# ashvardanian/StringWars

Measured on AMD Instinct MI355X. Metric: GCUPS (DP cell updates/s) batched Levenshtein, higher is better.
Workload: dtype u32; 1 GPU; C2 tokens64: 1000000 ASCII token pairs per GPU, lengths U[32,96], unbounded Levenshtein, tapes prepared and resident in HBM; step=one synchronous call (results visible on return), pairs_per_gpu=1000000, pairs_total=1000000, cells_per_gpu=4273938131, algorithm=auto, offsets=uint32, collective=none, seed=42

## Files before the change

### stringwars_amd/csrc/bp_item.hpp

```cpp
#pragma once
#include <type_traits>

#include "common.hpp"
#include "bp_window.hpp"

namespace swh {

struct SymWindow32 {
    const uint32_t *base;
    int lo, hi;
    __device__ __forceinline__ void init(const uint32_t *data, uint64_t start, uint64_t total) {
        auto c31 = [](int64_t v) { return (int)(v < -0x40000000ll ? -0x40000000ll : (v > 0x40000000ll ? 0x40000000ll : v)); };
        base = data + start;
        lo = c31(-(int64_t)start);
        hi = c31((int64_t)total - (int64_t)start - 1);
    }
    __device__ __forceinline__ uint32_t fetch(int idx) const { return base[bp_med3i(idx, lo, hi)]; }
    __device__ __forceinline__ void fetch4(int idx, uint32_t (&out)[4]) const {
        if (hi - lo >= 3) {
            const int c = bp_med3i(idx, lo, hi - 3);
            uint4 v;
            __builtin_memcpy(&v, base + c, 16);
            out[0] = v.x; out[1] = v.y; out[2] = v.z; out[3] = v.w;
            if (__builtin_expect(c == idx, 1)) return;
        }
#pragma unroll
        for (int q = 0; q < 4; ++q) out[q] = fetch(idx + q);
    }
};

template <typename Sym> struct BpTraits;
template <> struct BpTraits<uint8_t> {
    static constexpr int kWaves = 4, kEntries = 32, kMinWavesPerSimd = 4;
};
template <> struct BpTraits<uint32_t> {
    static constexpr int kWaves = 2, kEntries = 56, kMinWavesPerSimd = 2;
};
template <typename Sym> constexpr int bp_table_words() { return BpTraits<Sym>::kEntries * 64; }
template <typename Sym> constexpr size_t bp_lds_bytes() {
    return (size_t)BpTraits<Sym>::kWaves * (bp_table_words<Sym>() + 64) * 4 + 80 * 4;
}

struct GroupTables3 {
    uint32_t tbase, mask;
    __device__ __forceinline__ void init(uint32_t *table, int lane) {
        tbase = (uint32_t)(uintptr_t)(lds_u32 *)(table + lane);
        if (tbase & 0x700u) __builtin_trap();
        mask = 0x700u;
        asm volatile("" : "+v"(mask));
    }
    template <int G> __device__ __forceinline__ uint32_t addr(uint32_t c) const {
        uint32_t s;
        if constexpr (3 * G <= 8) s = c << (8 - 3 * G);
        else s = c >> (3 * G - 8);
        return (uint32_t)__builtin_amdgcn_bitop3_b32((int)s, (int)mask, (int)tbase, 0xEA);
    }
    __device__ __forceinline__ uint32_t lookup(uint32_t c) const { return lookup_n<7>(c); }
    __device__ __forceinline__ void insert(uint32_t c, uint32_t bit) const { insert_n<7>(c, bit); }
    template <int NG, int G> __device__ __forceinline__ uint32_t entry_n(uint32_t c) const {
        if constexpr (G + 1 == NG && NG < 7) {
            uint32_t idx = c >> (3 * G);
            idx = idx < 8u ? idx : 8u;
            return *(const lds_u32 *)(uintptr_t)(tbase + (idx << 8) + 2048u * G);
        } else {
            return *(const lds_u32 *)(uintptr_t)(addr<G>(c) + 2048u * G);
        }
    }
    template <int NG> __device__ __forceinline__ uint32_t lookup_n(uint32_t c) const {
        uint32_t e = entry_n<NG, 0>(c) & entry_n<NG, 1>(c);
        e &= entry_n<NG, 2>(c) & entry_n<NG, 3>(c);
        if constexpr (NG > 4) e &= entry_n<NG, 4>(c);
        if constexpr (NG > 5) e &= entry_n<NG, 5>(c);
        if constexpr (NG > 6) e &= entry_n<NG, 6>(c);
        return e;
    }
    template <int NG> __device__ __forceinline__ void insert_n(uint32_t c, uint32_t bit) const {
        __hip_atomic_fetch_or((lds_u32 *)(uintptr_t)addr<0>(c), bit, __ATOMIC_RELAXED, __HIP_MEMORY_SCOPE_WORKGROUP);
        __hip_atomic_fetch_or((lds_u32 *)(uintptr_t)(addr<1>(c) + 2048), bit, __ATOMIC_RELAXED, __HIP_MEMORY_SCOPE_WORKGROUP);
        __hip_atomic_fetch_or((lds_u32 *)(uintptr_t)(addr<2>(c) + 4096), bit, __ATOMIC_RELAXED, __HIP_MEMORY_SCOPE_WORKGROUP);
        __hip_atomic_fetch_or((lds_u32 *)(uintptr_t)(addr<3>(c) + 6144), bit, __ATOMIC_RELAXED, __HIP_MEMORY_SCOPE_WORKGROUP);
        if constexpr (NG > 4) __hip_atomic_fetch_or((lds_u32 *)(uintptr_t)(addr<4>(c) + 8192), bit, __ATOMIC_RELAXED, __HIP_MEMORY_SCOPE_WORKGROUP);
        if constexpr (NG > 5) __hip_atomic_fetch_or((lds_u32 *)(uintptr_t)(addr<5>(c) + 10240), bit, __ATOMIC_RELAXED, __HIP_MEMORY_SCOPE_WORKGROUP);
        if constexpr (NG > 6) __hip_atomic_fetch_or((lds_u32 *)(uintptr_t)(addr<6>(c) + 12288), bit, __ATOMIC_RELAXED, __HIP_MEMORY_SCOPE_WORKGROUP);
    }
};

template <typename Sym>
struct BpWave {
    static constexpr bool kBytes = sizeof(Sym) == 1;
    uint32_t *table;
    uint32_t *acc;
    NibbleTables nib;
    GroupTables3 grp;
    int lane;
    uint64_t a_total, b_total;
    __device__ __forceinline__ void init(uint32_t *table_, uint32_t *acc_, int lane_, uint64_t a_total_, uint64_t b_total_) {
        table = table_; acc = acc_; lane = lane_; a_total = a_total_; b_total = b_total_;
        if constexpr (kBytes) nib.init(table, lane);
        else grp.init(table, lane);
#pragma unroll
        for (int k = 0; k < BpTraits<Sym>::kEntries; ++k) table[k * 64 + lane] = 0;
    }
};

template <typename Sym, bool kWide>
__device__ __forceinline__ void bp_item(const KernelArgs &args, BpWave<Sym> &wv, const uint32_t G, const bool have, const uint64_t p,
                                        const uint64_t a0, const uint32_t la, const uint64_t b0, const uint32_t lb,
                                        uint16_t *staged = nullptr, const uint64_t staged_base = 0) {
    constexpr bool kBytes = sizeof(Sym) == 1;
    constexpr bool wide_tapes = kWide;
    const int lane = wv.lane;
    uint32_t *const table = wv.table;
    uint32_t *const acc = wv.acc;
    [[maybe_unused]] const NibbleTables &nib = wv.nib;
    [[maybe_unused]] const GroupTables3 &grp = wv.grp;
    const uint64_t a_total = wv.a_total, b_total = wv.b_total;
    const uint32_t slot = (uint32_t)lane / G, blk = (uint32_t)lane - slot * G;
    const bool a_is_pattern = bp_pattern_is_a(la, lb);
    const uint32_t m = a_is_pattern ? la : lb, n = a_is_pattern ? lb : la;
    using Window = typename std::conditional<kBytes, ByteWindow, SymWindow32>::type;
    Window pat, txt;
    pat.init((const Sym *)(a_is_pattern ? args.job.a.data : args.job.b.data), a_is_pattern ? a0 : b0,
             a_is_pattern ? a_total : b_total);
    txt.init((const Sym *)(a_is_pattern ? args.job.b.data : args.job.a.data), a_is_pattern ? b0 : a0,
             a_is_pattern ? b_total : a_total);

    const uint32_t row0 = blk * 32;
    const uint32_t brows = have ? (m > row0 ? (m - row0 < 32 ? m - row0 : 32) : 0) : 0;

    constexpr int kTextRegs = kBytes ? 4 : 16;
    uint32_t tnxt[kTextRegs];
    int tshift[kBytes ? 4 : 1];
    auto fetch_text = [&](int first) {
        if constexpr (kBytes) {
            if (wide_tapes) {
                tshift[0] = txt.fetch16_raw(first, tnxt);
            } else {
#pragma unroll
                for (int q = 0; q < 4; ++q) tnxt[q] = txt.fetch4_raw(first + q * 4, tshift[q]);
            }
        } else {
#pragma unroll
            for (int q = 0; q < 16; q += 4) {
                uint32_t four[4];
                txt.fetch4(first + q, four);
#pragma unroll
                for (int r = 0; r < 4; ++r) tnxt[q + r] = four[r];
            }
        }
    };
    fetch_text(0 - (int)blk);
    [[maybe_unused]] uint32_t groups = 7;

    if constexpr (kBytes) {
        uint32_t praw[8];
        int pshift[8];
        if (wide_tapes) {
            uint32_t half[2][4];
            const int moved0 = pat.fetch16_raw((int)row0, half[0]), moved1 = pat.fetch16_raw((int)row0 + 16, half[1]);
            pat.fix16((int)row0, moved0, half[0]);
            pat.fix16((int)row0 + 16, moved1, half[1]);
#pragma unroll
            for (int q = 0; q < 8; ++q) { praw[q] = half[q >> 2][q & 3]; pshift[q] = 24; }
        } else {
#pragma unroll
            for (int q = 0; q < 8; ++q) praw[q] = pat.fetch4_raw((int)row0 + q * 4, pshift[q]);
        }
        const uint32_t row_mask = brows >= 32 ? 0xFFFFFFFFu : ((1u << brows) - 1u);
#pragma unroll
        for (int q = 0; q < 8; ++q) {
            if (brows > (uint32_t)q * 4) {
                const uint32_t dw = ByteWindow::realign(praw[q], pshift[q]);
                nib.template insert<0>(dw, row_mask & (1u << (q * 4 + 0)));
                nib.template insert<1>(dw, row_mask & (1u << (q * 4 + 1)));
                nib.template insert<2>(dw, row_mask & (1u << (q * 4 + 2)));
                nib.template insert<3>(dw, row_mask & (1u << (q * 4 + 3)));
            }
        }
    } else {
        uint32_t psym[32];
#pragma unroll
        for (int q = 0; q < 32; q += 4) {
            uint32_t four[4];
            pat.fetch4((int)row0 + q, four);
#pragma unroll
            for (int r = 0; r < 4; ++r) psym[q + r] = four[r];
        }
        uint32_t seen = 0;
#pragma unroll
        for (int q = 0; q < 32; ++q) seen |= (uint32_t)q < brows ? psym[q] : 0u;
#pragma unroll
        for (int off = 32; off >= 1; off >>= 1) seen |= (uint32_t)__shfl_xor((int)seen, off);
        groups = seen < (1u << 12) ? 4u : (seen < (1u << 15) ? 5u : (seen < (1u << 18) ? 6u : 7u));
        auto enter = [&](auto ng_tag) {
            constexpr int NG = decltype(ng_tag)::value;
#pragma unroll
            for (int q = 0; q < 32; ++q)
                if ((uint32_t)q < brows) grp.template insert_n<NG>(psym[q], 1u << q);
        };
        if (groups == 4) enter(std::integral_constant<int, 4>{});
        else if (groups == 5) enter(std::integral_constant<int, 5>{});
        else if (groups == 6) enter(std::integral_constant<int, 6>{});
        else enter(std::integral_constant<int, 7>{});
    }
    acc[lane] = 0;
    wave_lds_fence();

    const uint32_t n_eff = wave_max_u32(have ? n + G - 1 : 0);
    const uint32_t steps = (n_eff + 15) & ~15u;

    const bool first_blk = blk == 0;
    uint32_t keep_mask = first_blk ? 0u : 0xFFFFFFFFu, first_ph = first_blk ? 0x80000000u : 0u;
    asm volatile("" : "+v"(keep_mask), "+v"(first_ph));
    uint32_t pv = 0xFFFFFFFFu, mv = 0, ph = 0, mh = 0;
    auto column = [&](uint32_t eq, uint32_t s) {
        uint32_t ph_in = (uint32_t)__builtin_amdgcn_update_dpp(0, (int)ph, 0x138, 0xf, 0xf, true);
        uint32_t mh_in = (uint32_t)__builtin_amdgcn_update_dpp(0, (int)mh, 0x138, 0xf, 0xf, true);
        ph_in = (uint32_t)__builtin_amdgcn_bitop3_b32((int)ph_in, (int)keep_mask, (int)first_ph, 0xEA);
        mh_in = mh_in & keep_mask;
        if (s - blk < n) {
            uint32_t xv = eq | mv;
            eq |= mh_in >> 31;
            uint32_t xh = (((eq & pv) + pv) ^ pv) | eq;
            ph = mv | ~(xh | pv);
            mh = pv & xh;
            uint32_t ph_s = __builtin_amdgcn_alignbit(ph, ph_in, 31);
            uint32_t mh_s = __builtin_amdgcn_alignbit(mh, mh_in, 31);
            pv = mh_s | ~(xv | ph_s);
            mv = ph_s & xv;
        }
    };
    auto columns = [&](auto ng_tag) {
    [[maybe_unused]] constexpr int NG = decltype(ng_tag)::value;
    for (uint32_t s0 = 0; s0 < steps; s0 += 16) {
        uint32_t tcur[kTextRegs];
        if constexpr (kBytes) {
            if (wide_tapes) {
#pragma unroll
                for (int q = 0; q < 4; ++q) tcur[q] = tnxt[q];
                txt.fix16((int)s0 - (int)blk, tshift[0], tcur);
            } else {
#pragma unroll
                for (int q = 0; q < 4; ++q) tcur[q] = ByteWindow::realign(tnxt[q], tshift[q]);
            }
        } else {
#pragma unroll
            for (int q = 0; q < kTextRegs; ++q) tcur[q] = tnxt[q];
        }
        fetch_text((int)s0 + 16 - (int)blk);
#pragma unroll
        for (int q = 0; q < 4; ++q) {
            const uint32_t gs = s0 + q * 4;
            if (gs >= n_eff) break;
            uint32_t eqs[4];
            if constexpr (kBytes) {
                eqs[0] = nib.template lookup<0>(tcur[q]);
                eqs[1] = nib.template lookup<1>(tcur[q]);
                eqs[2] = nib.template lookup<2>(tcur[q]);
                eqs[3] = nib.template lookup<3>(tcur[q]);
            } else {
#pragma unroll
                for (int u = 0; u < 4; ++u) eqs[u] = grp.template lookup_n<NG>(tcur[q * 4 + u]);
            }
#pragma unroll
            for (int u = 0; u < 4; ++u) column(eqs[u], gs + u);
        }
    }
    };
    if constexpr (kBytes) columns(std::integral_constant<int, 7>{});
    else if (groups == 4) columns(std::integral_constant<int, 4>{});
    else if (groups == 5) columns(std::integral_constant<int, 5>{});
    else if (groups == 6) columns(std::integral_constant<int, 6>{});
    else columns(std::integral_constant<int, 7>{});

    const uint32_t mask = brows >= 32 ? 0xFFFFFFFFu : ((1u << brows) - 1u);
    int part = __popc(pv & mask) - __popc(mv & mask);
    if (have && brows) atomicAdd(&acc[slot * G], (uint32_t)part);
    wave_lds_fence();
    if (have && first_blk) {
        uint32_t d = n + acc[lane];
        const uint32_t bounded = clamp_bound(d, args.job.bound);
        if (staged && bounded < 0xFFFFu) staged[p - staged_base] = (uint16_t)bounded;
        else store_result(args.job, p, (int64_t)bounded);
    }
    if constexpr (kBytes) {
#pragma unroll
        for (int k = 0; k < BpTraits<Sym>::kEntries; ++k) table[k * 64 + lane] = 0;
    } else {
#pragma unroll
        for (int k = 0; k < 32; ++k) table[k * 64 + lane] = 0;
        if (groups > 4) {
#pragma unroll
            for (int k = 32; k < BpTraits<Sym>::kEntries; ++k) table[k * 64 + lane] = 0;
        }
    }
    wave_lds_fence();
}

}
```

Measured before the change: 30780 GCUPS.

## Software-pipeline LDS nibble lookups one group ahead in byte Levenshtein loop

For byte-alphabet inputs, the column loop is restructured so the LDS nibble-table loads for the next four text bytes are issued before the bit-parallel column updates of the current four. Even and odd register buffers alternate, and text refill and realign happen every 16 columns. The goal is to hide LDS latency behind the dependent ALU chain of the Myers update. The cost is more live registers, which may reduce occupancy, plus more intricate index bookkeeping.

New measurement: 31150 GCUPS, median of 5. +1.2%, better.

```diff
diff --git a/stringwars_amd/csrc/bp_item.hpp b/stringwars_amd/csrc/bp_item.hpp
--- a/stringwars_amd/csrc/bp_item.hpp
+++ b/stringwars_amd/csrc/bp_item.hpp
@@ -207,7 +207,7 @@
     wave_lds_fence();
 
     const uint32_t n_eff = wave_max_u32(have ? n + G - 1 : 0);
-    const uint32_t steps = (n_eff + 15) & ~15u;
+    [[maybe_unused]] const uint32_t steps = (n_eff + 15) & ~15u;
 
     const bool first_blk = blk == 0;
     uint32_t keep_mask = first_blk ? 0u : 0xFFFFFFFFu, first_ph = first_blk ? 0x80000000u : 0u;
@@ -231,43 +231,82 @@
         }
     };
     auto columns = [&](auto ng_tag) {
-    [[maybe_unused]] constexpr int NG = decltype(ng_tag)::value;
-    for (uint32_t s0 = 0; s0 < steps; s0 += 16) {
-        uint32_t tcur[kTextRegs];
+        if constexpr (!kBytes) {
+            constexpr int NG = decltype(ng_tag)::value;
+            for (uint32_t s0 = 0; s0 < steps; s0 += 16) {
+                uint32_t tcur[kTextRegs];
+#pragma unroll
+                for (int q = 0; q < kTextRegs; ++q) tcur[q] = tnxt[q];
+                fetch_text((int)s0 + 16 - (int)blk);
+#pragma unroll
+                for (int q = 0; q < 4; ++q) {
+                    const uint32_t gs = s0 + q * 4;
+                    if (gs >= n_eff) break;
+                    uint32_t eqs[4];
+#pragma unroll
+                    for (int u = 0; u < 4; ++u) eqs[u] = grp.template lookup_n<NG>(tcur[q * 4 + u]);
+#pragma unroll
+                    for (int u = 0; u < 4; ++u) column(eqs[u], gs + u);
+                }
+            }
+        }
+    };
+    auto columns_ahead = [&]() {
         if constexpr (kBytes) {
-            if (wide_tapes) {
-#pragma unroll
-                for (int q = 0; q < 4; ++q) tcur[q] = tnxt[q];
-                txt.fix16((int)s0 - (int)blk, tshift[0], tcur);
-            } else {
-#pragma unroll
-                for (int q = 0; q < 4; ++q) tcur[q] = ByteWindow::realign(tnxt[q], tshift[q]);
-            }
-        } else {
-#pragma unroll
-            for (int q = 0; q < kTextRegs; ++q) tcur[q] = tnxt[q];
-        }
-        fetch_text((int)s0 + 16 - (int)blk);
-#pragma unroll
-        for (int q = 0; q < 4; ++q) {
-            const uint32_t gs = s0 + q * 4;
-            if (gs >= n_eff) break;
-            uint32_t eqs[4];
-            if constexpr (kBytes) {
-                eqs[0] = nib.template lookup<0>(tcur[q]);
-                eqs[1] = nib.template lookup<1>(tcur[q]);
-                eqs[2] = nib.template lookup<2>(tcur[q]);
-                eqs[3] = nib.template lookup<3>(tcur[q]);
-            } else {
-#pragma unroll
-                for (int u = 0; u < 4; ++u) eqs[u] = grp.template lookup_n<NG>(tcur[q * 4 + u]);
-            }
-#pragma unroll
-            for (int u = 0; u < 4; ++u) column(eqs[u], gs + u);
-        }
-    }
+            const uint32_t iterations = (n_eff + 7) >> 3;
+            uint32_t tq[4];
+            auto refill = [&](int first) {
+                if (wide_tapes) {
+#pragma unroll
+                    for (int q = 0; q < 4; ++q) tq[q] = tnxt[q];
+                    txt.fix16(first, tshift[0], tq);
+                } else {
+#pragma unroll
+                    for (int q = 0; q < 4; ++q) tq[q] = ByteWindow::realign(tnxt[q], tshift[q]);
+                }
+                fetch_text(first + 16);
+            };
+            auto request = [&](uint32_t x, uint32_t (&w)[8]) {
+                w[0] = *(const lds_u32 *)(uintptr_t)nib.template lo_addr<0>(x);
+                w[1] = *(const lds_u32 *)(uintptr_t)(nib.template hi_addr<0>(x) + 4096);
+                w[2] = *(const lds_u32 *)(uintptr_t)nib.template lo_addr<1>(x);
+                w[3] = *(const lds_u32 *)(uintptr_t)(nib.template hi_addr<1>(x) + 4096);
+                w[4] = *(const lds_u32 *)(uintptr_t)nib.template lo_addr<2>(x);
+                w[5] = *(const lds_u32 *)(uintptr_t)(nib.template hi_addr<2>(x) + 4096);
+                w[6] = *(const lds_u32 *)(uintptr_t)nib.template lo_addr<3>(x);
+                w[7] = *(const lds_u32 *)(uintptr_t)(nib.template hi_addr<3>(x) + 4096);
+            };
+            auto group = [&](const uint32_t (&w)[8], uint32_t s) {
+                uint32_t eq[4];
+#pragma unroll
+                for (int u = 0; u < 4; ++u) eq[u] = w[2 * u] & w[2 * u + 1];
+                asm volatile("" : "+v"(eq[0]), "+v"(eq[1]), "+v"(eq[2]), "+v"(eq[3]));
+#pragma unroll
+                for (int u = 0; u < 4; ++u) column(eq[u], s + u);
+            };
+            uint32_t even[8], odd[8];
+            refill(0 - (int)blk);
+            request(tq[0], even);
+            tq[0] = tq[1]; tq[1] = tq[2]; tq[2] = tq[3];
+            for (uint32_t it = 0; it < iterations; ++it) {
+                const uint32_t s = it * 8;
+                request(tq[0], odd);
+                group(even, s);
+                uint32_t next;
+                if (it & 1u) {
+                    refill((int)(s + 8) - (int)blk);
+                    next = tq[0];
+                    tq[0] = tq[1]; tq[1] = tq[2]; tq[2] = tq[3];
+                } else {
+                    next = tq[1];
+                    tq[0] = tq[2];
+                }
+                request(next, even);
+                group(odd, s + 4);
+            }
+        }
     };
-    if constexpr (kBytes) columns(std::integral_constant<int, 7>{});
+    if constexpr (kBytes) columns_ahead();
     else if (groups == 4) columns(std::integral_constant<int, 4>{});
     else if (groups == 5) columns(std::integral_constant<int, 5>{});
     else if (groups == 6) columns(std::integral_constant<int, 6>{});
```
